# xissburg/edyn

Hardware: AMD Instinct MI355X
Metric: steps/sec (whole node), 32k-box pile, 10 SI iters; HBM GB/s in solve (higher is better)
Workload: dtype f32

## Files before the change

edyn_amd/csrc/capi.hip:

```cpp
#include "ctx.hpp"
#include "dpolyhedron.hpp"
#include <algorithm>
#include <atomic>
#include <chrono>
#include <cstdio>
#include <cstring>

namespace eh {
using namespace dm;

static std::string g_create_error;

int set_error(edynhip_ctx *c, int code, const char *what, hipError_t e) {
    std::string msg = what ? what : "";
    if (e != hipSuccess) { msg += ": "; msg += hipGetErrorString(e); }
    if (c) c->err = msg; else g_create_error = msg;
    return code;
}

__global__ void k_publish_counters(const uint32_t *__restrict__ src, uint32_t *dst, uint32_t words, volatile uint32_t *seq, uint32_t value) {
    for (uint32_t i = threadIdx.x; i < words; i += blockDim.x) dst[i] = src[i];
    __threadfence_system();
    __syncthreads();
    if (threadIdx.x == 0) { __hip_atomic_store((uint32_t *)seq, value, __ATOMIC_RELEASE, __HIP_MEMORY_SCOPE_SYSTEM); }
// ... 429 lines not shown
    const uint32_t i = list[t];
    const uint32_t fl = b.flags[i];
    if ((fl & BF_KIND_MASK) == EDYNHIP_KIND_DYNAMIC) wake[b.island[i]] = 1u;
    b.flags[i] = EDYNHIP_KIND_STATIC | BF_REMOVED;
    b.linvel[i] = make_float4(0, 0, 0, 0); b.angvel[i] = make_float4(0, 0, 0, 0);
    b.grav[i] = make_float4(0, 0, 0, 0);
    float4 p = B_POS(b, i); p.w = 0; B_POS(b, i) = p;
    B_DV(b, i) = make_float4(0, 0, 0, 0); B_DW(b, i) = make_float4(0, 0, 0, 0);
    b.island[i] = i;
}
__global__ void k_mark_touching(uint32_t n, const uint32_t *__restrict__ list, Bodies b, uint32_t *wake) {
    const uint32_t t = blockIdx.x * blockDim.x + threadIdx.x;
    if (t >= n) return;
    const uint32_t i = list[t];
    if ((b.flags[i] & BF_KIND_MASK) == EDYNHIP_KIND_DYNAMIC) wake[b.island[i]] = 1u;
}
__global__ void k_wake_partners(uint32_t M, Manifolds mf, Bodies b, uint32_t *wake) {
    const uint32_t m = blockIdx.x * blockDim.x + threadIdx.x;
    if (m >= M) return;
    const uint32_t a = mf.bodyA[m], bb = mf.bodyB[m];
    const bool ra = b.flags[a] & BF_REMOVED, rb = b.flags[bb] & BF_REMOVED;
    if (ra && (b.flags[bb] & BF_KIND_MASK) == EDYNHIP_KIND_DYNAMIC) wake[b.island[bb]] = 1u;
    if (rb && (b.flags[a] & BF_KIND_MASK) == EDYNHIP_KIND_DYNAMIC) wake[b.island[a]] = 1u;
}
__global__ void k_wake_marked(uint32_t n, Bodies b, uint32_t *wake, double *since) {
    const uint32_t i = blockIdx.x * blockDim.x + threadIdx.x;
    if (i >= n) return;
    const uint32_t fl = b.flags[i];
    if ((fl & BF_KIND_MASK) != EDYNHIP_KIND_DYNAMIC) return;
    const uint32_t l = b.island[i];
    if (wake[l]) { b.flags[i] = fl & ~BF_ASLEEP; if (l == i) since[i] = -1.0; }
}
static int index_scratch(edynhip_ctx *c, size_t count, uint32_t *&out) {
    if (count > c->idx_scratch_cap) {
        if (c->idx_scratch) (void)hipFree(c->idx_scratch);
        c->idx_scratch = nullptr; c->idx_scratch_cap = 0;
        const size_t cap = std::max<size_t>(count * 2, 1024);
        EH_HIP(c, hipMalloc((void **)&c->idx_scratch, cap * sizeof(uint32_t)));
        c->idx_scratch_cap = cap;
    }
    out = c->idx_scratch;
    return EDYNHIP_OK;
}
int wake_islands_of(edynhip_ctx *c, const std::vector<uint32_t> &bodies) {
    if (!c->sleeping || bodies.empty() || c->b.n == 0) { c->all_asleep = false; return EDYNHIP_OK; }
    uint32_t *list = nullptr;
    EH_TRY(index_scratch(c, bodies.size(), list));
    EH_HIP(c, hipMemcpyAsync(list, bodies.data(), bodies.size() * sizeof(uint32_t), hipMemcpyHostToDevice, c->stream));
    EH_HIP(c, hipMemsetAsync(c->sleep_action, 0, (size_t)c->b.n * sizeof(uint32_t), c->stream));
    hipLaunchKernelGGL(k_mark_touching, dim3(((uint32_t)bodies.size() + 127) / 128), dim3(128), 0, c->stream, (uint32_t)bodies.size(), list, c->b, c->sleep_action);
    hipLaunchKernelGGL(k_wake_marked, dim3((c->b.n + 255) / 256), dim3(256), 0, c->stream, c->b.n, c->b, c->sleep_action, c->sleep_since);
    hipError_t e = hipStreamSynchronize(c->stream);
    c->all_asleep = false;
    if (e != hipSuccess) return set_error(c, EDYNHIP_ERR_HIP, "wake_islands_of", e);
    return EDYNHIP_OK;
}

}

using namespace eh;

extern "C" {

uint32_t edynhip_abi_version(void) { return 15; }

const char *edynhip_last_error(const edynhip_ctx *ctx) { return ctx ? ctx->err.c_str() : g_create_error.c_str(); }

edynhip_ctx *edynhip_create(const edynhip_config *cfg, int *status_out) {
    auto fail = [&](int code, const char *msg, hipError_t e = hipSuccess) -> edynhip_ctx * {
        set_error(nullptr, code, msg, e);
        if (status_out) *status_out = code;
        return nullptr;
    };
    if (!cfg || cfg->max_bodies == 0) return fail(EDYNHIP_ERR_INVALID, "edynhip_create: bad config");
    int ndev = 0;
    hipError_t e = hipGetDeviceCount(&ndev);
    if (e != hipSuccess || ndev <= 0) return fail(EDYNHIP_ERR_NO_DEVICE, "edynhip_create: no HIP device (this library has no CPU fallback)", e);
    if (cfg->device < 0 || cfg->device >= ndev) return fail(EDYNHIP_ERR_INVALID, "edynhip_create: device ordinal out of range");
    e = hipSetDevice(cfg->device);
    if (e != hipSuccess) return fail(EDYNHIP_ERR_HIP, "hipSetDevice", e);
    edynhip_ctx *c = new edynhip_ctx();
    c->cfg = *cfg;
    c->sleeping = (cfg->flags & EDYNHIP_FLAG_SLEEPING) != 0;
    c->device = cfg->device;
    if (c->cfg.max_manifolds == 0) c->cfg.max_manifolds = 16 * c->cfg.max_bodies + 1024;
    if (c->cfg.fixed_dt <= 0) c->cfg.fixed_dt = 1.0f / 60.0f;
    e = hipStreamCreateWithFlags(&c->stream, hipStreamNonBlocking);
    if (e != hipSuccess) { delete c; return fail(EDYNHIP_ERR_HIP, "hipStreamCreate", e); }
    int rc = allocate(c);
    if (rc != EDYNHIP_OK) {
        g_create_error = c->err;
        if (status_out) *status_out = rc;
        edynhip_destroy(c);
        return nullptr;
    }
    if (status_out) *status_out = EDYNHIP_OK;
    return c;
}

void edynhip_destroy(edynhip_ctx *c) {
    if (!c) return;
    if (getenv("EDYNHIP_TREE_STATS"))
        fprintf(stderr, "[edynhip] island labels: %llu steps relabelled in full, %llu incrementally\n", (unsigned long long)c->cc_full_steps, (unsigned long long)c->cc_incremental_steps);
    (void)hipSetDevice(c->device);
    if (c->stream) (void)hipStreamSynchronize(c->stream);
    eh::raycast_free(c);
    eh::query_aabb_free(c);
    for (void *p : c->allocs) (void)hipFree(p);
    if (c->idx_scratch) (void)hipFree(c->idx_scratch);
    for (void *p : c->mesh_allocs) (void)hipFree(p);
    if (c->rot) (void)hipFree(c->rot);
    if (c->poly_work) (void)hipFree(c->poly_work);
    if (c->cnt_host) (void)hipHostFree(c->cnt_host);
    if (c->cnt_seq) (void)hipHostFree((void *)c->cnt_seq);
    if (c->state_host) (void)hipHostFree(c->state_host);
    for (int k = 0; k < 2; ++k) {
        if (c->snap_host[k]) (void)hipHostFree(c->snap_host[k]);
        if (c->snap_event[k]) (void)hipEventDestroy(c->snap_event[k]);
    }
    if (c->evp_host) (void)hipHostFree(c->evp_host);
    if (c->evp_np_done) (void)hipEventDestroy(c->evp_np_done);
    if (c->evp_ready) (void)hipEventDestroy(c->evp_ready);
    for (int k = 0; k < 2; ++k) {
        if (c->rec_host[k]) (void)hipHostFree(c->rec_host[k]);
        if (c->rec_event[k]) (void)hipEventDestroy(c->rec_event[k]);
    }
    if (c->snap_ready) (void)hipEventDestroy(c->snap_ready);
    if (c->snap_stream) (void)hipStreamDestroy(c->snap_stream);
    for (auto &e : c->timer.ev) (void)hipEventDestroy(e);
    if (c->own_stream && c->stream) (void)hipStreamDestroy(c->stream);
    delete c;
}

int edynhip_set_stream(edynhip_ctx *c, void *hip_stream) {
    if (!c) return EDYNHIP_ERR_INVALID;
    EH_HIP(c, hipStreamSynchronize(c->stream));
    if (c->own_stream && c->stream) (void)hipStreamDestroy(c->stream);
    if (hip_stream) { c->stream = (hipStream_t)hip_stream; c->own_stream = false; }
    else { EH_HIP(c, hipStreamCreateWithFlags(&c->stream, hipStreamNonBlocking)); c->own_stream = true; }
    return EDYNHIP_OK;
}

int edynhip_synchronize(edynhip_ctx *c) {
    if (!c) return EDYNHIP_ERR_INVALID;
    EH_HIP(c, hipStreamSynchronize(c->stream));
    return EDYNHIP_OK;
}

static int rebuild_broadphase_lists(edynhip_ctx *c) {
    std::vector<uint32_t> np_list, proc_list;
    for (uint32_t i = 0; i < (uint32_t)c->host_kind.size(); ++i) {
        if (c->host_shape[i] == EDYNHIP_SHAPE_NONE) continue;
        (c->host_kind[i] == EDYNHIP_KIND_DYNAMIC ? proc_list : np_list).push_back(i);
    }
    EH_HIP(c, hipMemsetAsync(c->own_count, 0, ((size_t)c->b.cap + 1) * sizeof(uint32_t), c->stream));
    c->all_asleep = false;
    c->bvh.age = 0;
    c->bvh.lists_dirty = true;
    ++c->state_epoch;
    c->bvh.num_np = (uint32_t)np_list.size();
    c->bvh.num_proc = (uint32_t)proc_list.size();
    np_list.insert(np_list.end(), proc_list.begin(), proc_list.end());
    if (!np_list.empty())
        EH_HIP(c, hipMemcpyAsync(c->bvh.np_list, np_list.data(), np_list.size() * sizeof(uint32_t), hipMemcpyHostToDevice, c->stream));
    EH_HIP(c, hipStreamSynchronize(c->stream));
    return EDYNHIP_OK;
// ... 1239 lines not shown
```

edyn_amd/csrc/ctx.hpp:

```cpp
#pragma once
#include <hip/hip_runtime.h>
#include <cstdint>
#include <string>
#include <array>
#include <map>
#include <vector>
#include "../../include/edynhip.h"
#include "dmesh.hpp"

namespace eh {

constexpr uint32_t kNoColour = 0xFFu;
constexpr uint32_t kMaxColours = 64;
constexpr uint32_t kMaxContactColours = 63;
constexpr uint32_t kSerialColour = 62;
constexpr int kMaxPts = 4;

constexpr uint32_t BF_KIND_MASK = 0x3u;
constexpr uint32_t BF_SHAPE_SHIFT = 4;
constexpr uint32_t BF_SHAPE_MASK = 0xF0u;
constexpr uint32_t BF_ASLEEP = 0x100u;
constexpr uint32_t BF_NOSLEEP = 0x200u;
constexpr uint32_t BF_REMOVED = 0x400u;
__host__ __device__ inline bool edge_asleep(uint32_t fa, uint32_t fb) {
// ... 185 lines not shown
    uint32_t recorded = 0;
    uint32_t capacity = 0;
    hipEvent_t *e = nullptr;
    uint32_t mask = 0;
};

#define B_POS(b, i) ((b).xf[8 * (size_t)(i)])
#define B_ORN(b, i) ((b).xf[8 * (size_t)(i) + 1])
#define B_IW(b, i, r) ((b).xf[8 * (size_t)(i) + 2 + (r)])
#define B_IL(b, i, r) ((b).xf[8 * (size_t)(i) + 5 + (r)])
#define B_ORG(b, i) (((b).origin && (b).com[(i)].w != 0.0f) ? from4((b).origin[(i)]) : from4(B_POS(b, i)))
#define B_DV(b, i) ((b).dvw[2 * (size_t)(i)])
#define B_DW(b, i) ((b).dvw[2 * (size_t)(i) + 1])

}

struct edynhip_ctx {
    edynhip_config cfg{};
    int device = 0;
    hipStream_t stream = nullptr;
    bool own_stream = true;
    std::string err;
    eh::Bodies b;
    eh::Manifolds m[2];
    int cur = 0;
    uint32_t num_manifolds = 0;
    eh::Joints j;
    std::vector<eh::HostJoint> host_joints;
    std::vector<uint32_t> pending_redefs;
    eh::Rows rows;
    eh::LBVH bvh;
    float4 *np_ra = nullptr, *np_rb = nullptr, *np_rn = nullptr;
    uint32_t *np_rnum = nullptr;
    uint64_t *pair_keys = nullptr, *pair_keys_sorted = nullptr;
    uint64_t *own_keys = nullptr;
    uint32_t *own_count = nullptr, *own_offset = nullptr;
    uint2 *new_edges = nullptr;
    uint32_t *new_edge_m = nullptr;
    uint32_t prev_num_manifolds = 0;
    uint32_t *col_keys = nullptr, *col_keys_sorted = nullptr;
    uint32_t *cs_hist = nullptr, *cs_start = nullptr;
    uint32_t *cs_sup = nullptr;
    uint32_t col_lds_edges = 0;
    uint64_t cc_full_steps = 0, cc_incremental_steps = 0;
    bool coop_launched = false;
    uint32_t col_lds_bytes = 0;
    uint32_t *col_unc = nullptr;
    uint64_t *used = nullptr;
    uint2 *isl_top = nullptr;
    uint64_t *best[2] = {nullptr, nullptr};
    float *pos_err = nullptr;
    float4 *com_store = nullptr, *origin_store = nullptr;
    uint32_t *isl_cnt = nullptr, *isl_off = nullptr, *isl_list = nullptr, *isl_items = nullptr, *isl_sorted = nullptr, *isl_joint = nullptr;
    uint32_t isl_prep_step = 0xFFFFFFF0u;
    uint32_t last_fetch_step = 0xFFFFFFF0u;
    uint32_t topology_epoch = 0;
    uint32_t isl_lists_epoch = 0xFFFFFFFFu;
    uint32_t isl_cache_epoch = 0xFFFFFFFFu, isl_cache_max = 0, isl_cache_free = 0, isl_cache_jmax = 0;
    float *isl_err = nullptr;
    uint32_t *isl_done = nullptr;
    void *sort_tmp = nullptr;
    size_t sort_tmp_bytes = 0;
    eh::Counters *cnt = nullptr;
    eh::Counters *cnt_host = nullptr;
    volatile uint32_t *cnt_seq = nullptr;
    uint32_t cnt_seq_next = 0;
    eh::StageTimer timer;
    edynhip_timings timings{};
    edynhip_stats stats{};
    uint32_t num_colours = 0;
    uint32_t colour_start[eh::kMaxColours] = {0}, colour_end[eh::kMaxColours] = {0};
    uint32_t colour_split[eh::kMaxColours][3] = {{0}};
    uint32_t num_active = 0;
    std::vector<void *> allocs;
    uint32_t *idx_scratch = nullptr; size_t idx_scratch_cap = 0;
    bool clears_primed = false;
    bool full_step = false;
    float *state_dev = nullptr;
    float *state_host = nullptr;
    bool sleeping = false;
    bool all_asleep = false;
    bool solve_begin_done = false;
    bool has_generic = false;
    bool has_cylinder = false;
    bool has_polyhedron = false;
    struct HostMeshes {
        std::vector<dc::MeshDesc> desc;
        std::vector<float4> vertices, normals, edge_vertices, edge_normals, relevant_normals;
        std::vector<uint32_t> face_first, edge_vidx, edge_faces, relevant_faces, relevant_edges, nb_start, nb_idx;
        void swap(HostMeshes &o) { std::swap(*this, o); }
    } host_meshes;
    dc::Meshes meshes;
    std::vector<void *> mesh_allocs;
    float4 *rot = nullptr; size_t rot_cap = 0, rot_used = 0;
    uint32_t *rot_off = nullptr;
    std::vector<uint32_t> host_rot_off;
    uint32_t *poly_work = nullptr;
    struct MixIdPair { uint32_t first, second; };
    struct MixIdPairLess {
        bool operator()(const MixIdPair &a, const MixIdPair &b) const {
            if (a.first == b.second && a.second == b.first) return false;
            if (a.first == b.first) return a.second < b.second;
            return a.first < b.first;
        }
    };
    std::map<MixIdPair, std::array<float, 6>, MixIdPairLess> host_mix;
    std::vector<uint32_t> host_mat_id;
    uint32_t *d_mat_cid = nullptr; int32_t *d_mix_lut = nullptr; float *d_mix_vals = nullptr; uint32_t mix_lut_cap = 0, mix_vals_cap = 0;
    bool extras = false;
    uint32_t step_index = 0;
    eh::ContactEvent *events = nullptr; uint32_t *event_count = nullptr; uint32_t event_cap = 0; uint8_t *prev_matched = nullptr;
    float *snap_host[2] = {nullptr, nullptr}; float *snap_dev[2] = {nullptr, nullptr}; hipEvent_t snap_event[2] = {nullptr, nullptr};
    uint32_t snap_step[2] = {0, 0}, snap_bodies[2] = {0, 0}; int snap_last = -1; hipStream_t snap_stream = nullptr; hipEvent_t snap_ready = nullptr;
    uint32_t num_sleepable = 0;
    bool sleep_active() const { return sleeping && num_sleepable > 0; }
    unsigned long long *pp_prof_dev = nullptr; int pp_prof_calls = 0;
    bool island_labels_valid = false;
    uint32_t excl_dirty_lo = 0xFFFFFFFFu, excl_dirty_hi = 0;
    uint32_t evp_max = 0; uint8_t *evp_host = nullptr; hipEvent_t evp_np_done = nullptr, evp_ready = nullptr; bool evp_now = false; int evp_state = 0;
    uint8_t *rec_host[2] = {nullptr, nullptr}; uint8_t *rec_dev[2] = {nullptr, nullptr}; hipEvent_t rec_event[2] = {nullptr, nullptr};
    uint32_t rec_step[2] = {0, 0}, rec_bodies[2] = {0, 0}, rec_events_copied[2] = {0, 0}; int rec_last = -1; uint32_t rec_event_cap = 0;
    double sim_clock = 0;
    int (*pair_filter)(void *, uint32_t, uint32_t) = nullptr;
    void *pair_filter_user = nullptr;
    uint32_t *filter_new_idx = nullptr;
    std::vector<uint64_t> host_group, host_mask;
    uint32_t *sleep_state = nullptr, *sleep_action = nullptr;
    double *sleep_since = nullptr;
    uint32_t *sleep_old_label = nullptr, *sleep_size = nullptr, sleep_prev_n = 0;
    unsigned long long *sleep_best = nullptr;
    double *sleep_carried = nullptr;
    int df_mode = -1;
    uint32_t df_lanes = 0;
    uint32_t dfp_waves = 0;
    uint32_t df2_waves = 0;
    uint32_t df4_waves = 0;
    bool inplace_step = false;
    bool points_in_prev = false;
    bool force_islands = true;
    bool has_restitution = false;
    uint32_t restitution_iterations = 8, individual_restitution_iterations = 3;
    uint32_t *rdeg = nullptr, *roff = nullptr, *rcursor = nullptr, *radj = nullptr, *rvisited = nullptr, *rqnext = nullptr;
    uint8_t *rstar = nullptr;
    uint64_t *rbest = nullptr;
    float4 *rimp = nullptr;
    uint32_t *excl = nullptr;
    std::vector<uint32_t> host_excl;
    std::vector<int32_t> host_kind, host_shape;
    uint64_t state_epoch = 1;
    eh::RayTree *ray = nullptr;
    eh::QueryAabb *qa = nullptr;
    bool world_shard = false;
    const uint32_t *answers = nullptr;
    std::vector<uint32_t> host_answers;
    const uint32_t *query_island = nullptr;
};

namespace eh {
int broadphase(edynhip_ctx *c);
int narrowphase(edynhip_ctx *c);
int count_points(edynhip_ctx *c);
int fetch_counters(edynhip_ctx *c, size_t bytes);
int publish_counters(edynhip_ctx *c, size_t bytes, uint32_t *ticket);
int wait_counters(edynhip_ctx *c, uint32_t ticket);
int scan_u32(edynhip_ctx *c, const uint32_t *in, uint32_t *out, uint32_t n);
int debug_collide(edynhip_ctx *c, uint32_t n, const int32_t *st, const float *sp, const float *pos, const float *orn, float threshold,
// ... 34 lines not shown
```

edyn_amd/csrc/narrowphase.hip:

```cpp
#include "ctx.hpp"
#include "dpolyhedron.hpp"

namespace eh {
using namespace dc;

struct BodyIn { f3 pos; q4 orn; f3 angvel; float friction, restitution; bool rolling; };

DI f3 local_normal(const CPoint &rp, const BodyIn &A, const BodyIn &B) {
    return rp.attachment != NA_NONE ? rotate(conjugate(rp.attachment == NA_ON_A ? A.orn : B.orn), rp.normal) : mk3(0, 0, 0);
}
DI int find_nearest(const CPoint &cp, const CPoint (&rs)[4], int R) {
    float best = square(kCachingThreshold);
    int idx = R;
#pragma unroll
    for (int i = 0; i < 4; ++i) {
        if (i < R) {
            float dA = length_sqr(rs[i].pivotA - cp.pivotA);
            float dB = length_sqr(rs[i].pivotB - cp.pivotB);
            if (dA < best) { best = dA; idx = i; }
            if (dB < best) { best = dB; idx = i; }
        }
    }
    return idx;
}
// ... 151 lines not shown
    st.rnum[m] = (uint32_t)res.num;
    for (int k = 0; k < res.num; ++k) {
        const size_t d = (size_t)k * mf.cap + m;
        st.ra[d] = to4(res.pt[k].pivotA, res.pt[k].distance);
        st.rb[d] = to4(res.pt[k].pivotB, __int_as_float(res.pt[k].attachment));
        st.rn[d] = to4(res.pt[k].normal, 0.0f);
    }
}

DI PPSide pp_side_of(const Meshes &meshes, const Bodies &b, uint32_t body) { return pp_side(meshes, b.shape[body], meshes.rot + meshes.rot_off[body]); }
template <int G, bool PROF>
__global__ void __launch_bounds__(64)
k_np_pp_axes(Manifolds mf, Bodies b, Staging st, Meshes meshes, PolyBins pb, unsigned long long *prof_out) {
    constexpr uint32_t kGroups = 64u / G;
    const uint32_t g = threadIdx.x / G;
    const uint32_t n = pb.start[kPolyPairBins];
    PPProf<PROF> prof;
    if (PROF) for (int k = 0; k < 8; ++k) prof.t[k] = 0;
    uint32_t iters = 0;
    for (uint32_t i = blockIdx.x * kGroups + g; i < n; i += gridDim.x * kGroups) {
        prof.stamp(0);
        const uint32_t m = pb.list[i];
        const uint32_t ia = mf.bodyA[m], ib = mf.bodyB[m];
        PPSeparation sep;
        const bool touching = pp_group_axes<G>(meshes, pp_side_of(meshes, b, ia), pp_side_of(meshes, b, ib), B_ORG(b, ib) - B_ORG(b, ia), kCollisionThreshold, sep, prof);
        if (threadIdx.x % G == 0) {
            pb.hint[m] = sep.hint;
            if (touching) {
                pb.key[atomicAdd(&pb.cursor[kPolyBins - 1], 1u)] = m;
                st.ra[m] = to4(sep.axis, sep.distance);
                st.rb[m] = make_float4(sep.projectionA, sep.projectionB, 0.0f, 0.0f);
            } else {
                st.rnum[m] = 0;
            }
        }
        prof.stamp(3);
        ++iters;
    }
    if (PROF && threadIdx.x % G == 0) {
        atomicAdd(&prof_out[0], (unsigned long long)iters);
        for (int k = 1; k < 4; ++k) atomicAdd(&prof_out[k], (unsigned long long)(prof.t[k] - prof.t[k - 1]));
    }
}
template <int G, bool PROF>
__global__ void __launch_bounds__(64)
k_np_pp_contacts(Manifolds mf, Bodies b, Staging st, Meshes meshes, PolyBins pb, unsigned long long *prof_out) {
    constexpr uint32_t kGroups = 64u / G;
    __shared__ __align__(16) unsigned char lds_raw[kGroups * sizeof(PPLds)];
    const uint32_t g = threadIdx.x / G;
    PPLds &lds = reinterpret_cast<PPLds *>(lds_raw)[g];
    const uint32_t n = pb.cursor[kPolyBins - 1];
    PPProf<PROF> prof;
    if (PROF) for (int k = 0; k < 8; ++k) prof.t[k] = 0;
    uint32_t iters = 0;
    for (uint32_t i = blockIdx.x * kGroups + g; i < n; i += gridDim.x * kGroups) {
        prof.stamp(2);
        const uint32_t m = pb.key[i];
        const uint32_t ia = mf.bodyA[m], ib = mf.bodyB[m];
        const float4 r0 = st.ra[m], r1 = st.rb[m];
        const PPSeparation sep{from4(r0), r0.w, r1.x, r1.y};
        CResult res;
        res.num = 0;
        const Ctx ctx{B_ORG(b, ia), q_from4(B_ORN(b, ia)), B_ORG(b, ib), q_from4(B_ORN(b, ib)), kCollisionThreshold};
        pp_group_contacts<G>(pp_side_of(meshes, b, ia), pp_side_of(meshes, b, ib), ctx, sep, lds, res, prof);
        if (threadIdx.x % G == 0) {
            st.rnum[m] = (uint32_t)res.num;
            for (int k = 0; k < res.num; ++k) {
                const size_t d = (size_t)k * mf.cap + m;
                st.ra[d] = to4(res.pt[k].pivotA, res.pt[k].distance);
                st.rb[d] = to4(res.pt[k].pivotB, __int_as_float(res.pt[k].attachment));
                st.rn[d] = to4(res.pt[k].normal, 0.0f);
            }
        }
        pp_group_sync();
        prof.stamp(6);
        ++iters;
    }
    if (PROF && threadIdx.x % G == 0) {
        atomicAdd(&prof_out[4], (unsigned long long)iters);
        for (int k = 3; k < 7; ++k) atomicAdd(&prof_out[k + 2], (unsigned long long)(prof.t[k] - prof.t[k - 1]));
    }
}

__global__ void __launch_bounds__(64, 2)
k_np_merge(uint32_t M, Manifolds mf, Bodies b, float dt, bool sleeping, Manifolds old, bool points_in_old, Staging st, EventSink ev) {
    const uint32_t m = blockIdx.x * blockDim.x + threadIdx.x;
    if (m < M) {
        const uint32_t ia = mf.bodyA[m], ib = mf.bodyB[m];
        const uint32_t info = mf.info[m];
        const int n_old = (int)(info & 0xFF);
        const uint32_t fa = b.flags[ia], fb = b.flags[ib];
        const Manifolds &src = points_in_old ? old : mf;
        const uint32_t sidx = points_in_old ? mf.prev_idx[m] : m;
        if (sleeping && edge_asleep(fa, fb)) {
            if (points_in_old)
                for (int k = 0; k < n_old; ++k) {
                    const size_t ts = pt_at(src.cap, (uint32_t)k, sidx), td = pt_at(mf.cap, (uint32_t)k, m);
                    mf.pA[td] = src.pA[ts]; mf.pB[td] = src.pB[ts]; mf.nrm[td] = src.nrm[ts]; mf.lnrm[td] = src.lnrm[ts]; mf.imp[td] = src.imp[ts];
                    const size_t s = slot_at(src.cap, (uint32_t)k, sidx), d = slot_at(mf.cap, (uint32_t)k, m);
                    if (mf.pid) mf.pid[d] = src.pid[s];
                    if (mf.xmat) { mf.xmat[d] = src.xmat[s]; mf.ximp[d] = src.ximp[s]; }
                }
            return;
        }
        const int tA = (int)((fa & BF_SHAPE_MASK) >> BF_SHAPE_SHIFT), tB = (int)((fb & BF_SHAPE_MASK) >> BF_SHAPE_SHIFT);
        BodyIn A, B;
        { A.pos = B_ORG(b, ia); A.orn = q_from4(B_ORN(b, ia)); A.angvel = from4(b.angvel[ia]);
          float2 mt = b.mat[ia]; A.friction = mt.x; A.restitution = mt.y;
          A.rolling = (fa & BF_KIND_MASK) == EDYNHIP_KIND_DYNAMIC && (tA == SHAPE_SPHERE || tA == SHAPE_CAPSULE || tA == SHAPE_CYLINDER); }
        { B.pos = B_ORG(b, ib); B.orn = q_from4(B_ORN(b, ib)); B.angvel = from4(b.angvel[ib]);
          float2 mt = b.mat[ib]; B.friction = mt.x; B.restitution = mt.y;
          B.rolling = (fb & BF_KIND_MASK) == EDYNHIP_KIND_DYNAMIC && (tB == SHAPE_SPHERE || tB == SHAPE_CAPSULE || tB == SHAPE_CYLINDER); }

        CPoint pts[kMaxPts];
#pragma unroll
        for (int k = 0; k < kMaxPts; ++k) {
            if (k < n_old) {
                const size_t s = pt_at(src.cap, (uint32_t)k, sidx);
                const float4 a = src.pA[s], bb = src.pB[s], n = src.nrm[s];
                CPoint &p = pts[k];
                p.pivotA = from4(a); p.pivotB = from4(bb); p.normal = from4(n); p.attachment = __float_as_int(n.w);
                p.distance = dot(p.normal, to_world(p.pivotA, A.pos, A.orn) - to_world(p.pivotB, B.pos, B.orn));
            } else {
                pts[k] = CPoint{};
            }
        }

        const int R = (int)st.rnum[m];
        CPoint rs[kMaxPts];
#pragma unroll
        for (int k = 0; k < kMaxPts; ++k) {
            if (k < R) {
                const size_t d = (size_t)k * mf.cap + m;
                const float4 ra = st.ra[d], rb = st.rb[d], rn = st.rn[d];
                rs[k] = CPoint{from4(ra), from4(rb), from4(rn), ra.w, __float_as_int(rb.w)};
            } else {
                rs[k] = CPoint{};
            }
        }

        uint32_t merged = 0, dead = 0, changed = 0;
        int num_points = n_old;
#pragma unroll
        for (int i = 0; i < kMaxPts; ++i) {
            if (i < n_old) {
                CPoint &cp = pts[i];
                int nearest = find_nearest(cp, rs, R);
                if (nearest == R && A.rolling) nearest = find_nearest_rolling(rs, R, cp.pivotA, A.pos, A.orn, A.angvel, dt);
                if (nearest == R && B.rolling) nearest = find_nearest_rolling(rs, R, cp.pivotB, B.pos, B.orn, B.angvel, dt);
                if (nearest < R && !((merged >> nearest) & 1u)) { cp = pick4(rs, nearest); changed |= 1u << i; merged |= 1u << nearest; }
                else if (should_remove(cp, A, B)) { dead |= 1u << i; --num_points; }
            }
        }
        const uint32_t all_r = (1u << R) - 1u;

        CPoint lp[kMaxPts];
        uint32_t create = 0;
        if ((merged & all_r) != all_r) {
            int lold[kMaxPts] = {-1, -1, -1, -1};
            int ltype[kMaxPts] = {INS_NONE, INS_NONE, INS_NONE, INS_NONE};
#pragma unroll
            for (int i = 0; i < kMaxPts; ++i) lp[i] = CPoint{};
            if (num_points > 0) {
                int k = 0;
#pragma unroll
                for (int i = 0; i < kMaxPts; ++i) {
                    if (i < n_old && !((dead >> i) & 1u)) {
                        CPoint loc = pts[i];
                        loc.attachment = NA_NONE;
                        put4(lp, k, loc);
                        put4(lold, k, i);
                        ++k;
                    }
                }
            } else {
                num_points = 1;
                lp[0] = rs[0];
                ltype[0] = INS_APPEND;
                merged |= 1u;
            }
#pragma unroll
            for (int r = 0; r < kMaxPts; ++r) {
                if (r < R && !((merged >> r) & 1u)) {
                    const CPoint rp = rs[r];
                    f3 piv[kMaxPts];
#pragma unroll
                    for (int i = 0; i < kMaxPts; ++i) piv[i] = lp[i].pivotA;
                    int ir = insertion_point_index(piv, num_points, rp.pivotA);
                    if ((ir & 0xFF) == INS_NONE) {
#pragma unroll
                        for (int i = 0; i < kMaxPts; ++i) piv[i] = lp[i].pivotB;
                        ir = insertion_point_index(piv, num_points, rp.pivotB);
                    }
                    if ((ir & 0xFF) != INS_NONE) { put4(lp, ir >> 8, rp); put4(ltype, ir >> 8, ir & 0xFF); }
                }
            }
#pragma unroll
            for (int i = 0; i < kMaxPts; ++i) {
                if (i < num_points) {
                    const int ty = ltype[i], lo = lold[i];
                    if (ty == INS_APPEND || (ty == INS_SIMILAR && lo < 0)) create |= 1u << i;
                    else if (ty == INS_SIMILAR) {
#pragma unroll
                        for (int j = 0; j < kMaxPts; ++j) sel(pts[j], j == lo, lp[i]);
                        changed |= 1u << lo;
                    } else if (ty == INS_REPLACE) {
                        if (lo >= 0) dead |= 1u << lo;
                        create |= 1u << i;
                    }
                }
            }
        }
        float4 ext_l[kMaxPts], ext_i[kMaxPts];
        float ext_f[kMaxPts];
        uint64_t ext_id[kMaxPts] = {0, 0, 0, 0};
        if (mf.pid) {
#pragma unroll
            for (int i = 0; i < kMaxPts; ++i) {
                if (i < n_old) {
                    ext_id[i] = src.pid[(size_t)i * src.cap + sidx];
                    if ((dead >> i) & 1u) emit_event(ev, EDYNHIP_EVENT_POINT_DESTROYED, ia, ib, ext_id[i]);
                }
            }
        }
#pragma unroll
        for (int i = 0; i < kMaxPts; ++i) {
            if (i < n_old && !((dead >> i) & 1u)) {
                const size_t s = pt_at(src.cap, (uint32_t)i, sidx);
                ext_l[i] = src.lnrm[s]; ext_i[i] = src.imp[s]; ext_f[i] = src.pB[s].w;
            } else {
                ext_l[i] = ext_i[i] = make_float4(0, 0, 0, 0); ext_f[i] = 0;
            }
        }
        int n_out = 0;
        if (create) {
            float friction = sqrtf(A.friction * B.friction);
            float restitution = fminf(A.restitution, B.restitution);
            if (const float *e = mix_lookup(b, ia, ib)) { restitution = e[0]; friction = e[1]; }
#pragma unroll
            for (int i = kMaxPts - 1; i >= 0; --i) {
                if ((create >> i) & 1u) {
                    const CPoint &p = lp[i];
                    const size_t d = pt_at(mf.cap, (uint32_t)n_out, m);
                    mf.pA[d] = to4(p.pivotA, p.distance);
                    mf.pB[d] = to4(p.pivotB, friction);
                    mf.nrm[d] = to4(p.normal, __int_as_float(p.attachment));
                    mf.lnrm[d] = to4(local_normal(p, A, B), restitution);
                    mf.imp[d] = make_float4(0, 0, 0, __uint_as_float(0u));
                    if (mf.pid) {
                        const uint64_t id = ((uint64_t)(ev.step + 1u) << 32) | ((uint64_t)m << 2) | (uint64_t)i;
                        mf.pid[slot_at(mf.cap, (uint32_t)n_out, m)] = id;
                        emit_event(ev, EDYNHIP_EVENT_POINT_CREATED, ia, ib, id);
                    }
                    ++n_out;
                }
            }
        }
#pragma unroll
        for (int i = 0; i < kMaxPts; ++i) {
            if (i < n_old && !((dead >> i) & 1u)) {
                const CPoint &p = pts[i];
                const size_t d = pt_at(mf.cap, (uint32_t)n_out, m);
                const f3 ln = ((changed >> i) & 1u) ? local_normal(p, A, B) : from4(ext_l[i]);
                mf.pA[d] = to4(p.pivotA, p.distance);
                mf.pB[d] = to4(p.pivotB, ext_f[i]);
                mf.nrm[d] = to4(p.normal, __int_as_float(p.attachment));
                mf.lnrm[d] = to4(ln, ext_l[i].w);
                mf.imp[d] = make_float4(ext_i[i].x, ext_i[i].y, ext_i[i].z, __uint_as_float(__float_as_uint(ext_i[i].w) + 1u));
                if (mf.pid) mf.pid[slot_at(mf.cap, (uint32_t)n_out, m)] = ext_id[i];
                ++n_out;
            }
        }
        if (mf.xmat) {
            float4 xm[kMaxPts], xi[kMaxPts];
#pragma unroll
            for (int i = 0; i < kMaxPts; ++i) {
                if (i < n_old && !((dead >> i) & 1u)) { const size_t s = (size_t)i * src.cap + sidx; xm[i] = src.xmat[s]; xi[i] = src.ximp[s]; }
                else { xm[i] = xi[i] = make_float4(0, 0, 0, 0); }
            }
            const float4 ma = b.mat2[ia], mb = b.mat2[ib];
            float stiff = kLarge, damp = kLarge;
            if (ma.z < kLarge || mb.z < kLarge) { stiff = 1.0f / (1.0f / ma.z + 1.0f / mb.z); damp = 1.0f / (1.0f / ma.w + 1.0f / mb.w); }
            float4 fresh = make_float4(fmaxf(ma.y, mb.y), fmaxf(ma.x, mb.x), stiff, damp);
            if (const float *e = mix_lookup(b, ia, ib)) fresh = make_float4(e[3], e[2], e[4], e[5]);
            int slot = 0;
#pragma unroll
            for (int i = kMaxPts - 1; i >= 0; --i) if ((create >> i) & 1u) { const size_t d = (size_t)slot * mf.cap + m; mf.xmat[d] = fresh; mf.ximp[d] = make_float4(0, 0, 0, 0); ++slot; }
#pragma unroll
            for (int i = 0; i < kMaxPts; ++i) if (i < n_old && !((dead >> i) & 1u)) { const size_t d = (size_t)slot * mf.cap + m; mf.xmat[d] = xm[i]; mf.ximp[d] = xi[i]; ++slot; }
        }
        uint32_t colour = info >> 8;
        if (n_out == 0) colour = kNoColour;
        mf.info[m] = (uint32_t)n_out | (colour << 8);
    }
}

__global__ void k_count_points(uint32_t M, const uint32_t *__restrict__ info, Counters *cnt) {
    uint32_t m = blockIdx.x * blockDim.x + threadIdx.x;
    uint32_t pts = m < M ? (info[m] & 0xFF) : 0, act = pts ? 1u : 0u;
#pragma unroll
    for (int off = 32; off > 0; off >>= 1) { pts += __shfl_xor(pts, off); act += __shfl_xor(act, off); }
    if ((threadIdx.x & 63) == 0 && pts) { atomicAdd(&cnt->num_points, pts); atomicAdd(&cnt->num_active, act); }
}
int count_points(edynhip_ctx *c) {
    EH_HIP(c, hipMemsetAsync(&c->cnt->num_points, 0, 2 * sizeof(uint32_t), c->stream));
    const uint32_t M = c->num_manifolds;
    if (M) hipLaunchKernelGGL(k_count_points, dim3((M + 255) / 256), dim3(256), 0, c->stream, M, c->m[c->cur].info, c->cnt);
    EH_HIP(c, hipGetLastError());
    return EDYNHIP_OK;
}

template <bool EXT>
__global__ void __launch_bounds__(64, EXT ? 1 : 2) k_debug_collide(uint32_t n, const int32_t *__restrict__ st, const float4 *__restrict__ sp, const float *__restrict__ pos,
                                const float4 *__restrict__ orn, float threshold, float *out, uint32_t *count) {
    uint32_t i = blockIdx.x * blockDim.x + threadIdx.x;
    if (i >= n) return;
    Ctx ctx{mk3(pos[6 * i], pos[6 * i + 1], pos[6 * i + 2]), q_from4(orn[2 * i]), mk3(pos[6 * i + 3], pos[6 * i + 4], pos[6 * i + 5]),
            q_from4(orn[2 * i + 1]), threshold};
    CResult r;
    if (EXT) { r.num = 0; if (!collide_ext(st[2 * i], sp[2 * i], st[2 * i + 1], sp[2 * i + 1], ctx, r)) return; }
    else collide(st[2 * i], sp[2 * i], st[2 * i + 1], sp[2 * i + 1], ctx, r);
    count[i] = (uint32_t)r.num;
    for (int k = 0; k < r.num; ++k) {
        float *o = out + ((size_t)i * 4 + k) * 11;
        o[0] = r.pt[k].pivotA.x; o[1] = r.pt[k].pivotA.y; o[2] = r.pt[k].pivotA.z;
        o[3] = r.pt[k].pivotB.x; o[4] = r.pt[k].pivotB.y; o[5] = r.pt[k].pivotB.z;
        o[6] = r.pt[k].normal.x; o[7] = r.pt[k].normal.y; o[8] = r.pt[k].normal.z;
        o[9] = r.pt[k].distance; o[10] = (float)r.pt[k].attachment;
    }
}
__global__ void __launch_bounds__(64)
k_debug_collide_poly(uint32_t first, uint32_t n, const int32_t *__restrict__ st, const float4 *__restrict__ sp, const float *__restrict__ pos,
                     const float4 *__restrict__ orn, float threshold, float *out, uint32_t *count, Meshes meshes, float4 *scratch, uint32_t stride, int group) {
    const uint32_t i = first + blockIdx.x;
    if (blockIdx.x >= n) return;
    const int tA = st[2 * i], tB = st[2 * i + 1];
    if (tA != SHAPE_POLYHEDRON && tB != SHAPE_POLYHEDRON) return;
    float4 *rot[2] = {scratch + (size_t)(2 * blockIdx.x) * stride, scratch + (size_t)(2 * blockIdx.x + 1) * stride};
    for (int side = 0; side < 2; ++side) {
        if (st[2 * i + side] != SHAPE_POLYHEDRON) continue;
        const MeshDesc d = meshes.desc[(uint32_t)sp[2 * i + side].x];
        const q4 q = q_from4(orn[2 * i + side]) * q4{0, 0, 0, 1};
        for (uint32_t k = threadIdx.x; k < d.rot_size; k += 64) rotate_mesh_item(meshes, d, q, rot[side], k);
    }
    __syncthreads();
    Ctx ctx{mk3(pos[6 * i], pos[6 * i + 1], pos[6 * i + 2]), q_from4(orn[2 * i]), mk3(pos[6 * i + 3], pos[6 * i + 4], pos[6 * i + 5]),
            q_from4(orn[2 * i + 1]), threshold};
    CResult r;
    r.num = 0;
    if (group != 0 && tA == SHAPE_POLYHEDRON && tB == SHAPE_POLYHEDRON) {
        __shared__ __align__(16) unsigned char lds_raw[sizeof(PPLds)];
        PPLds &lds = *reinterpret_cast<PPLds *>(lds_raw);
        if ((int)threadIdx.x >= group) return;
        PPProf<false> noprof;
        const PPSide A = pp_side(meshes, sp[2 * i], rot[0]), B = pp_side(meshes, sp[2 * i + 1], rot[1]);
        PPSeparation sep;
        if (group == 16) { if (pp_group_axes<16>(meshes, A, B, ctx.posB - ctx.posA, ctx.threshold, sep, noprof)) pp_group_contacts<16>(A, B, ctx, sep, lds, r, noprof); }
        else if (group == 4) { if (pp_group_axes<4>(meshes, A, B, ctx.posB - ctx.posA, ctx.threshold, sep, noprof)) pp_group_contacts<4>(A, B, ctx, sep, lds, r, noprof); }
        else if (pp_group_axes<8>(meshes, A, B, ctx.posB - ctx.posA, ctx.threshold, sep, noprof)) pp_group_contacts<8>(A, B, ctx, sep, lds, r, noprof);
        if (threadIdx.x != 0) return;
    } else {
        if (threadIdx.x != 0) return;
        collide_poly(meshes, tA, sp[2 * i], rot[0], tB, sp[2 * i + 1], rot[1], ctx, r);
    }
    count[i] = (uint32_t)r.num;
    for (int k = 0; k < r.num; ++k) {
        float *o = out + ((size_t)i * 4 + k) * 11;
        o[0] = r.pt[k].pivotA.x; o[1] = r.pt[k].pivotA.y; o[2] = r.pt[k].pivotA.z;
        o[3] = r.pt[k].pivotB.x; o[4] = r.pt[k].pivotB.y; o[5] = r.pt[k].pivotB.z;
        o[6] = r.pt[k].normal.x; o[7] = r.pt[k].normal.y; o[8] = r.pt[k].normal.z;
        o[9] = r.pt[k].distance; o[10] = (float)r.pt[k].attachment;
    }
}
int debug_collide(edynhip_ctx *c, uint32_t n, const int32_t *st, const float *sp, const float *pos, const float *orn, float threshold,
                  float *out, uint32_t *count) {
    if (n == 0) return EDYNHIP_OK;
    const size_t b_st = (size_t)n * 8, b_sp = (size_t)n * 32, b_pos = (size_t)n * 24, b_orn = (size_t)n * 32, b_out = (size_t)n * 44 * 4, b_cnt = (size_t)n * 4;
    auto up16 = [](size_t x) { return (x + 15) & ~(size_t)15; };
    const size_t o_sp = up16(b_st), o_pos = o_sp + up16(b_sp), o_orn = o_pos + up16(b_pos), o_out = o_orn + up16(b_orn), o_cnt = o_out + up16(b_out);
    char *d = nullptr;
    EH_HIP(c, hipMalloc((void **)&d, o_cnt + up16(b_cnt)));
    hipStream_t s = c->stream;
    hipError_t e = hipMemcpyAsync(d, st, b_st, hipMemcpyHostToDevice, s);
    if (e == hipSuccess) e = hipMemcpyAsync(d + o_sp, sp, b_sp, hipMemcpyHostToDevice, s);
    if (e == hipSuccess) e = hipMemcpyAsync(d + o_pos, pos, b_pos, hipMemcpyHostToDevice, s);
    if (e == hipSuccess) e = hipMemcpyAsync(d + o_orn, orn, b_orn, hipMemcpyHostToDevice, s);
    if (e == hipSuccess) e = hipMemsetAsync(d + o_out, 0, b_out, s);
    if (e == hipSuccess) {
        hipLaunchKernelGGL(k_debug_collide<false>, dim3((n + 63) / 64), dim3(64), 0, s, n, (const int32_t *)d, (const float4 *)(d + o_sp), (const float *)(d + o_pos),
                           (const float4 *)(d + o_orn), threshold, (float *)(d + o_out), (uint32_t *)(d + o_cnt));
        bool any_cyl = false;
        for (uint32_t i = 0; i < 2 * n && !any_cyl; ++i) any_cyl = st[i] == EDYNHIP_SHAPE_CYLINDER;
        if (any_cyl)
            hipLaunchKernelGGL(k_debug_collide<true>, dim3((n + 63) / 64), dim3(64), 0, s, n, (const int32_t *)d, (const float4 *)(d + o_sp), (const float *)(d + o_pos),
                               (const float4 *)(d + o_orn), threshold, (float *)(d + o_out), (uint32_t *)(d + o_cnt));
        bool any_poly = false;
        for (uint32_t i = 0; i < 2 * n; ++i)
            if (st[i] == EDYNHIP_SHAPE_POLYHEDRON) {
                any_poly = true;
                const float id = sp[4 * i];
                if (!(id >= 0) || id >= (float)c->host_meshes.desc.size()) { (void)hipStreamSynchronize(s); (void)hipFree(d); return set_error(c, EDYNHIP_ERR_INVALID, "edynhip_debug_collide: unknown mesh id"); }
            }
        if (any_poly) {
            uint32_t stride = 0;
            for (const MeshDesc &md : c->host_meshes.desc) stride = std::max(stride, md.rot_size);
            const uint32_t chunk = 16384;
            const int group = getenv("EDYNHIP_POLY_GROUP") ? atoi(getenv("EDYNHIP_POLY_GROUP")) : 8;
            float4 *scratch = nullptr;
            e = hipMalloc((void **)&scratch, (size_t)chunk * 2 * stride * sizeof(float4));
            for (uint32_t first = 0; first < n && e == hipSuccess; first += chunk) {
                const uint32_t cnt = std::min(chunk, n - first);
                hipLaunchKernelGGL(k_debug_collide_poly, dim3(cnt), dim3(64), 0, s, first, cnt, (const int32_t *)d, (const float4 *)(d + o_sp), (const float *)(d + o_pos),
                                   (const float4 *)(d + o_orn), threshold, (float *)(d + o_out), (uint32_t *)(d + o_cnt), c->meshes, scratch, stride, group);
            }
            if (e == hipSuccess) e = hipStreamSynchronize(s);
            if (scratch) (void)hipFree(scratch);
        }
        if (e == hipSuccess) e = hipMemcpyAsync(out, d + o_out, b_out, hipMemcpyDeviceToHost, s);
    }
    if (e == hipSuccess) e = hipMemcpyAsync(count, d + o_cnt, b_cnt, hipMemcpyDeviceToHost, s);
    if (e == hipSuccess) e = hipStreamSynchronize(s);
    (void)hipFree(d);
    if (e != hipSuccess) return set_error(c, EDYNHIP_ERR_HIP, "edynhip_debug_collide", e);
    return EDYNHIP_OK;
}

int narrowphase(edynhip_ctx *c) {
    const uint32_t M = c->num_manifolds;
    if (M == 0) return EDYNHIP_OK;
    const Staging st{c->np_ra, c->np_rb, c->np_rn, c->np_rnum};
    hipLaunchKernelGGL(k_np_detect, dim3((M + 63) / 64), dim3(64), 0, c->stream, M, c->m[c->cur], c->b, c->sleeping, st);
    if (c->has_cylinder) hipLaunchKernelGGL(k_np_detect_ext, dim3((M + 63) / 64), dim3(64), 0, c->stream, M, c->m[c->cur], c->b, c->sleeping, st);
    if (c->has_polyhedron) {
        EH_TRY(update_rotated(c));
        uint32_t *pw = c->poly_work;
        const size_t cap = c->m[0].cap;
        uint32_t *const hints = pw + 3 * kPolyBins + 1 + 2 * cap;
        const PolyBins pb{pw, pw + kPolyBins, pw + 2 * kPolyBins, pw + 3 * kPolyBins, pw + 3 * kPolyBins + 1, pw + 3 * kPolyBins + 1 + cap, hints + (size_t)c->cur * cap};
        static const bool use_hints = !(getenv("EDYNHIP_POLY_HINT") && getenv("EDYNHIP_POLY_HINT")[0] == '0');
        hipLaunchKernelGGL(k_poly_count, dim3((M + 255) / 256), dim3(256), 0, c->stream, M, c->m[c->cur], c->b, c->sleeping, pb, c->meshes, hints + (size_t)(c->cur ^ 1) * cap,
                           !c->inplace_step, use_hints);
        hipLaunchKernelGGL(k_poly_scan, dim3(1), dim3(1024), 0, c->stream, pb);
        hipLaunchKernelGGL(k_poly_scatter, dim3((M + 255) / 256), dim3(256), 0, c->stream, M, pb);
        static const int group = getenv("EDYNHIP_POLY_GROUP") ? atoi(getenv("EDYNHIP_POLY_GROUP")) : 8;
        if (group != 0) {
            const uint32_t waves = 5120;
            static const int group2 = getenv("EDYNHIP_POLY_GROUP2") ? atoi(getenv("EDYNHIP_POLY_GROUP2")) : 4;
            static const bool prof = getenv("EDYNHIP_PP_PROF") != nullptr;
            unsigned long long *&prof_dev = c->pp_prof_dev;
            int &prof_calls = c->pp_prof_calls;
            if (prof && !prof_dev) { void *q = nullptr; EH_HIP(c, hipMalloc(&q, 128)); c->allocs.push_back(q); prof_dev = (unsigned long long *)q; EH_HIP(c, hipMemsetAsync(prof_dev, 0, 128, c->stream)); }
            const Manifolds &mfc = c->m[c->cur];
            unsigned long long *const pd = prof ? prof_dev : nullptr;
            if (prof) {
                if (group == 16) hipLaunchKernelGGL((k_np_pp_axes<16, true>), dim3(waves), dim3(64), 0, c->stream, mfc, c->b, st, c->meshes, pb, pd);
                else hipLaunchKernelGGL((k_np_pp_axes<8, true>), dim3(waves), dim3(64), 0, c->stream, mfc, c->b, st, c->meshes, pb, pd);
                if (group2 == 8) hipLaunchKernelGGL((k_np_pp_contacts<8, true>), dim3(waves), dim3(64), 0, c->stream, mfc, c->b, st, c->meshes, pb, pd);
                else hipLaunchKernelGGL((k_np_pp_contacts<4, true>), dim3(waves), dim3(64), 0, c->stream, mfc, c->b, st, c->meshes, pb, pd);
            } else {
                if (group == 16) hipLaunchKernelGGL((k_np_pp_axes<16, false>), dim3(waves), dim3(64), 0, c->stream, mfc, c->b, st, c->meshes, pb, pd);
                else hipLaunchKernelGGL((k_np_pp_axes<8, false>), dim3(waves), dim3(64), 0, c->stream, mfc, c->b, st, c->meshes, pb, pd);
                if (group2 == 8) hipLaunchKernelGGL((k_np_pp_contacts<8, false>), dim3(waves), dim3(64), 0, c->stream, mfc, c->b, st, c->meshes, pb, pd);
                else if (group2 == 16) hipLaunchKernelGGL((k_np_pp_contacts<16, false>), dim3(waves), dim3(64), 0, c->stream, mfc, c->b, st, c->meshes, pb, pd);
                else hipLaunchKernelGGL((k_np_pp_contacts<4, false>), dim3(waves), dim3(64), 0, c->stream, mfc, c->b, st, c->meshes, pb, pd);
            }
            if (prof && ++prof_calls % 100 == 0) {
                unsigned long long h[16];
                EH_HIP(c, hipMemcpyAsync(h, prof_dev, 128, hipMemcpyDeviceToHost, c->stream));
                EH_HIP(c, hipStreamSynchronize(c->stream));
                EH_HIP(c, hipMemsetAsync(prof_dev, 0, 128, c->stream));
                const double p = 100.0 * (double)std::max<unsigned long long>(h[0], 1), q = 100.0 * (double)std::max<unsigned long long>(h[4], 1);
                fprintf(stderr, "[pp prof, G=%d/%d] pairs/step %.0f, us per pair-iteration: setup+faces %.2f edges %.2f stores+wait %.2f; survivors/step %.0f: setup+polygons %.2f hulls %.2f contacts %.2f stores+wait %.2f\n",
                        group, group2, h[0] / 100.0, h[1] / p, h[2] / p, h[3] / p, h[4] / 100.0, h[5] / q, h[6] / q, h[7] / q, h[8] / q);
            }
        }
        hipLaunchKernelGGL(k_np_detect_poly, dim3((M + 63) / 64), dim3(64), 0, c->stream, M, c->m[c->cur], c->b, st, c->meshes, pb, group != 0);
    }
    hipLaunchKernelGGL(k_np_merge, dim3((M + 63) / 64), dim3(64), 0, c->stream, M, c->m[c->cur], c->b, c->cfg.fixed_dt, c->sleeping, c->m[c->cur ^ 1], c->points_in_prev, st, event_sink(c));
    c->points_in_prev = false;
    EH_HIP(c, hipGetLastError());
    return EDYNHIP_OK;
}

}
```

Measured before the change: 794.8.

## Fuse narrowphase detection and manifold merge into one kernel via LDS staging

Adds a k_np_contacts kernel that runs primitive collision detection and then the manifold merge in the same thread. Contact points are parked in shared memory instead of the global staging arrays. Pairs involving cylinders or polyhedra still take the old staged path, handled by a filtered k_np_merge launch. This is meant to remove one kernel launch and the global write/read round trip of raw contact points for box piles. In exchange, the fused kernel needs more LDS and registers, which may lower occupancy.

```diff
diff --git a/edyn_amd/csrc/capi.hip b/edyn_amd/csrc/capi.hip
--- a/edyn_amd/csrc/capi.hip
+++ b/edyn_amd/csrc/capi.hip
@@ -535,6 +535,7 @@
     edynhip_ctx *c = new edynhip_ctx();
     c->cfg = *cfg;
     c->sleeping = (cfg->flags & EDYNHIP_FLAG_SLEEPING) != 0;
+    c->np_fused = !(getenv("EDYNHIP_NP_FUSED") && getenv("EDYNHIP_NP_FUSED")[0] == '0');
     c->device = cfg->device;
     if (c->cfg.max_manifolds == 0) c->cfg.max_manifolds = 16 * c->cfg.max_bodies + 1024;
     if (c->cfg.fixed_dt <= 0) c->cfg.fixed_dt = 1.0f / 60.0f;
diff --git a/edyn_amd/csrc/ctx.hpp b/edyn_amd/csrc/ctx.hpp
--- a/edyn_amd/csrc/ctx.hpp
+++ b/edyn_amd/csrc/ctx.hpp
@@ -291,6 +291,7 @@
     bool all_asleep = false;
     bool solve_begin_done = false;
     bool has_generic = false;
+    bool np_fused = true;
     bool has_cylinder = false;
     bool has_polyhedron = false;
     struct HostMeshes {
diff --git a/edyn_amd/csrc/narrowphase.hip b/edyn_amd/csrc/narrowphase.hip
--- a/edyn_amd/csrc/narrowphase.hip
+++ b/edyn_amd/csrc/narrowphase.hip
@@ -257,10 +257,28 @@
     }
 }
 
-__global__ void __launch_bounds__(64, 2)
-k_np_merge(uint32_t M, Manifolds mf, Bodies b, float dt, bool sleeping, Manifolds old, bool points_in_old, Staging st, EventSink ev) {
-    const uint32_t m = blockIdx.x * blockDim.x + threadIdx.x;
-    if (m < M) {
+struct StagedResult {
+    Staging st; size_t cap; uint32_t m;
+    DI int num() const { return (int)st.rnum[m]; }
+    DI CPoint point(int k) const {
+        const size_t d = (size_t)k * cap + m;
+        const float4 ra = st.ra[d], rb = st.rb[d], rn = st.rn[d];
+        return CPoint{from4(ra), from4(rb), from4(rn), ra.w, __float_as_int(rb.w)};
+    }
+};
+constexpr int kNpLdsQuads = 3 * kMaxPts;
+struct LdsResult {
+    const float4 *q; const int *n;
+    DI int num() const { return *n; }
+    DI CPoint point(int k) const {
+        const float4 ra = q[(3 * k) * 64], rb = q[(3 * k + 1) * 64], rn = q[(3 * k + 2) * 64];
+        return CPoint{from4(ra), from4(rb), from4(rn), ra.w, __float_as_int(rb.w)};
+    }
+};
+
+template <class Result>
+DI void np_merge_lane(const uint32_t m, const Manifolds &mf, const Bodies &b, float dt, bool sleeping, const Manifolds &old, bool points_in_old, const Result &raw, const EventSink &ev) {
+    {
         const uint32_t ia = mf.bodyA[m], ib = mf.bodyB[m];
         const uint32_t info = mf.info[m];
         const int n_old = (int)(info & 0xFF);
@@ -301,17 +319,12 @@
             }
         }
 
-        const int R = (int)st.rnum[m];
+        const int R = raw.num();
         CPoint rs[kMaxPts];
 #pragma unroll
         for (int k = 0; k < kMaxPts; ++k) {
-            if (k < R) {
-                const size_t d = (size_t)k * mf.cap + m;
-                const float4 ra = st.ra[d], rb = st.rb[d], rn = st.rn[d];
-                rs[k] = CPoint{from4(ra), from4(rb), from4(rn), ra.w, __float_as_int(rb.w)};
-            } else {
-                rs[k] = CPoint{};
-            }
+            if (k < R) rs[k] = raw.point(k);
+            else rs[k] = CPoint{};
         }
 
         uint32_t merged = 0, dead = 0, changed = 0;
@@ -468,6 +481,58 @@
         if (n_out == 0) colour = kNoColour;
         mf.info[m] = (uint32_t)n_out | (colour << 8);
     }
+}
+
+DI bool np_staged_pair(uint32_t fa, uint32_t fb) {
+    const int tA = (int)((fa & BF_SHAPE_MASK) >> BF_SHAPE_SHIFT), tB = (int)((fb & BF_SHAPE_MASK) >> BF_SHAPE_SHIFT);
+    return tA == SHAPE_CYLINDER || tB == SHAPE_CYLINDER || tA == SHAPE_POLYHEDRON || tB == SHAPE_POLYHEDRON;
+}
+
+__global__ void __launch_bounds__(64, 2)
+k_np_merge(uint32_t M, Manifolds mf, Bodies b, float dt, bool sleeping, Manifolds old, bool points_in_old, Staging st, EventSink ev, bool staged_only) {
+    const uint32_t m = blockIdx.x * blockDim.x + threadIdx.x;
+    if (m >= M) return;
+    if (staged_only && !np_staged_pair(b.flags[mf.bodyA[m]], b.flags[mf.bodyB[m]])) return;
+    np_merge_lane(m, mf, b, dt, sleeping, old, points_in_old, StagedResult{st, mf.cap, m}, ev);
+}
+
+__global__ void __launch_bounds__(64, 2)
+k_np_contacts(uint32_t M, Manifolds mf, Bodies b, float dt, bool sleeping, Manifolds old, bool points_in_old, uint32_t *rnum, EventSink ev, bool staged_world) {
+    __shared__ float4 park[kNpLdsQuads * 64];
+    __shared__ int park_num[64];
+    const uint32_t m = blockIdx.x * blockDim.x + threadIdx.x;
+    float4 *const mine = park + threadIdx.x;
+    int num = -1;
+    if (m < M) {
+        const uint32_t ia = mf.bodyA[m], ib = mf.bodyB[m];
+        const uint32_t fa = b.flags[ia], fb = b.flags[ib];
+        if (staged_world && np_staged_pair(fa, fb)) {
+            rnum[m] = 0;
+        } else {
+            num = 0;
+            if (!(sleeping && edge_asleep(fa, fb))) {
+                const box3 ba{from4(b.amin[ia]), from4(b.amax[ia])}, bbx{from4(b.amin[ib]), from4(b.amax[ib])};
+                if (intersect(inset(ba, -kBreakingThreshold), bbx)) {
+                    const int tA = (int)((fa & BF_SHAPE_MASK) >> BF_SHAPE_SHIFT), tB = (int)((fb & BF_SHAPE_MASK) >> BF_SHAPE_SHIFT);
+                    Ctx ctx{B_ORG(b, ia), q_from4(B_ORN(b, ia)), B_ORG(b, ib), q_from4(B_ORN(b, ib)), kCollisionThreshold};
+                    CResult res;
+                    res.num = 0;
+                    collide(tA, b.shape[ia], tB, b.shape[ib], ctx, res);
+                    num = res.num;
+#pragma unroll
+                    for (int k = 0; k < kMaxPts; ++k) {
+                        if (k >= res.num) break;
+                        mine[(3 * k) * 64] = to4(res.pt[k].pivotA, res.pt[k].distance);
+                        mine[(3 * k + 1) * 64] = to4(res.pt[k].pivotB, __int_as_float(res.pt[k].attachment));
+                        mine[(3 * k + 2) * 64] = to4(res.pt[k].normal, 0.0f);
+                    }
+                }
+            }
+        }
+    }
+    park_num[threadIdx.x] = num;
+    __syncthreads();
+    if (park_num[threadIdx.x] >= 0) np_merge_lane(m, mf, b, dt, sleeping, old, points_in_old, LdsResult{mine, &park_num[threadIdx.x]}, ev);
 }
 
 __global__ void k_count_points(uint32_t M, const uint32_t *__restrict__ info, Counters *cnt) {
@@ -604,7 +669,12 @@
     const uint32_t M = c->num_manifolds;
     if (M == 0) return EDYNHIP_OK;
     const Staging st{c->np_ra, c->np_rb, c->np_rn, c->np_rnum};
-    hipLaunchKernelGGL(k_np_detect, dim3((M + 63) / 64), dim3(64), 0, c->stream, M, c->m[c->cur], c->b, c->sleeping, st);
+    const bool staged_world = c->has_cylinder || c->has_polyhedron;
+    if (c->np_fused)
+        hipLaunchKernelGGL(k_np_contacts, dim3((M + 63) / 64), dim3(64), 0, c->stream, M, c->m[c->cur], c->b, c->cfg.fixed_dt, c->sleeping, c->m[c->cur ^ 1], c->points_in_prev, c->np_rnum,
+                           event_sink(c), staged_world);
+    else
+        hipLaunchKernelGGL(k_np_detect, dim3((M + 63) / 64), dim3(64), 0, c->stream, M, c->m[c->cur], c->b, c->sleeping, st);
     if (c->has_cylinder) hipLaunchKernelGGL(k_np_detect_ext, dim3((M + 63) / 64), dim3(64), 0, c->stream, M, c->m[c->cur], c->b, c->sleeping, st);
     if (c->has_polyhedron) {
         EH_TRY(update_rotated(c));
@@ -651,7 +721,9 @@
         }
         hipLaunchKernelGGL(k_np_detect_poly, dim3((M + 63) / 64), dim3(64), 0, c->stream, M, c->m[c->cur], c->b, st, c->meshes, pb, group != 0);
     }
-    hipLaunchKernelGGL(k_np_merge, dim3((M + 63) / 64), dim3(64), 0, c->stream, M, c->m[c->cur], c->b, c->cfg.fixed_dt, c->sleeping, c->m[c->cur ^ 1], c->points_in_prev, st, event_sink(c));
+    if (!c->np_fused || staged_world)
+        hipLaunchKernelGGL(k_np_merge, dim3((M + 63) / 64), dim3(64), 0, c->stream, M, c->m[c->cur], c->b, c->cfg.fixed_dt, c->sleeping, c->m[c->cur ^ 1], c->points_in_prev, st, event_sink(c),
+                           c->np_fused);
     c->points_in_prev = false;
     EH_HIP(c, hipGetLastError());
     return EDYNHIP_OK;
```

Measured after the change: 815.2, median of 6. +2.6%, better.
